# SciML/NeuralPDE.jl

Hardware: AMD Instinct MI355X
Metric: collocation-point residual+grad evals/sec, 2D Poisson 4x64 MLP (higher is better)
Workload: dtype f32, hidden-layer forward / dA / dW GEMMs as 3-piece bf16 split products (6 bf16 MFMAs per product block, fp32 accumulation; 24 mantissa bits rebuilt; the five small piece products on an accumulator of their own: zero-mean, a third of the rms error of an fp32-MFMA fmaf chain per GEMM output, tools/m

## Files before the change

### neuralpde.jl_amd/csrc/pinn_kernels2.hpp

```cpp
#pragma once
#include "pinn_kernels.hpp"

#if defined(PINN_STAMP) && !defined(PINN_EMU)
#define STAMP_MEMBERS unsigned st_acc[24]; unsigned long long st_last;
#define STAMP_INIT(ac) { for (int i_ = 0; i_ < 24; ++i_) (ac).st_acc[i_] = 0; (ac).st_last = __builtin_amdgcn_s_memtime(); }
#define STAMP(i) { const unsigned long long st_now = __builtin_amdgcn_s_memtime(); ac.st_acc[i] += (unsigned)(st_now - ac.st_last); ac.st_last = st_now; }
#define STAMP_EXTRA 128
#else
#define STAMP_MEMBERS
#define STAMP_INIT(ac)
#define STAMP(i)
#define STAMP_EXTRA 0
#endif

#ifndef PINN_F2_REC_LDS
#define PINN_F2_REC_LDS 1
#endif
#ifndef PINN_F2_SWP
#define PINN_F2_SWP 7
#endif
#ifndef PINN_PROBE
#define PINN_PROBE 0
#endif
#ifndef PINN_F2_ADJ_IL
// ... 23 lines not shown

template <class A, class B> struct same_type { static constexpr bool value = false; };
template <class A> struct same_type<A, A> { static constexpr bool value = true; };
template <int HP_, int NHH_, int D_, int NW_, bool WBAR_REG_>
struct Shape2 {
    static constexpr int HP = HP_, MT = HP_ / 16, NHH = NHH_, LH = NHH_ + 1, D = D_, NW = NW_, MTW = MT / NW_;
    static constexpr bool WBAR_REG = WBAR_REG_;
};
template <class SH>
struct Acc2 {
    vfloat4 wbar[(SH::WBAR_REG && SH::NHH > 0) ? SH::NHH : 1][SH::MTW][SH::MT];
    vfloat4 bbar[SH::LH][SH::MTW];
    vfloat4 w1bar[SH::D][SH::MTW];
    vfloat4 wLbar[SH::MTW];
    vfloat bLbar;
    vfloat pbar[MAX_PARAMS];
    vdacc lsum;
    int cur_term;
    STAMP_MEMBERS
};

template <int HP_, int NHH_, int D_, unsigned D1MASK_, unsigned long long PAIRS_, int NPAIR_, int PG_, unsigned HI_ = 0, int GEMM_ = GEMM_SPLIT>
struct Spec2 {
    using J = JetSet<D1MASK_, PAIRS_, NPAIR_, HI_>;
    static constexpr unsigned HI = HI_;
    static constexpr int FAMILY = 2;
    static constexpr int GEMM = GEMM_;
    static constexpr int HP = HP_, MT = HP_ / 16, NHH = NHH_, LH = NHH_ + 1, D = D_, NPAIR = NPAIR_, PG = PG_;
    static constexpr unsigned D1MASK = D1MASK_;
    static constexpr unsigned long long PAIRS = PAIRS_;
    static constexpr int NW = (HP_ >= 128 && J::C * PG_ <= F2_NW8_MAXNG) ? F2_WAVES128 : 4;
// ... 39 lines not shown
    static constexpr int XSZB = BFX ? XSZ_BF : XSZ;
    static constexpr bool BFX_TR = BFX && TR_SHAPE;
    static constexpr bool DW_NATURAL = BFX_TR;
    static constexpr int ZTW = BFX_TR ? 0 : NG * (MT / NW) * 256;
    static constexpr int LDS_UP = (((NW + 1) * NG * 16 + 63) / 64) * 64;
    static_assert(PG_ >= 1 && PG_ <= 4, "one tape wave per point group");
    static constexpr bool CHUNKED = (2 * XSZB + NW * ZTW + LDS_UP) * 4 > 160 * 1024;
    static constexpr int CH_AT = 16 * HP_;
    static constexpr int CH_ZT = MTW * 256;
    static constexpr int CHSZ = CH_AT + NW * CH_ZT;
    static_assert(!CHUNKED || 2 * CHSZ <= XSZ, "chunk double buffer must fit inside X1");
    static constexpr int OFF_X1 = XSZB;
    static constexpr int OFF_ZT = 2 * XSZB;
    static constexpr int OFF_UP = 2 * XSZB + (CHUNKED ? 0 : NW * ZTW);
    static constexpr int LDS_BASE = OFF_UP + LDS_UP;
#ifndef PINN_F2_WG3
#define PINN_F2_WG3 0
#endif
    static constexpr int WG_PER_CU = (NW == 8) ? 1 : ((PINN_F2_WG3 && LDS_BASE * 4 <= 53 * 1024) ? 3 : ((LDS_BASE * 4 <= 80 * 1024) ? 2 : 1));
    static constexpr int RECQ = MT * 256;
    static constexpr int LDS_CAP = (WG_PER_CU == 3 ? 53 : (WG_PER_CU == 2 ? 80 : 160)) * 256 - 64;
    static constexpr int NRQ_ALL = (LH > 2 ? LH - 2 : 0) * NG;
    static constexpr int NRQ_FIT = (LDS_CAP - LDS_BASE) / RECQ;
    static constexpr int NRQ = PINN_F2_REC_LDS ? (NRQ_FIT < NRQ_ALL ? (NRQ_FIT > 0 ? NRQ_FIT : 0) : NRQ_ALL) : 0;
    static constexpr int LDS_WG = LDS_BASE + NRQ * RECQ;
    static constexpr int OCC = WG_PER_CU * NW / 4;
    static constexpr int LDS_FWD = 2 * XSZB + LDS_UP;
    static constexpr int WG_FWD_LDS = (160 * 1024 - 1024) / (LDS_FWD * 4);
    static constexpr int WG_FWD = (WG_FWD_LDS * NW >= 16) ? 16 / NW : (WG_FWD_LDS < 1 ? 1 : WG_FWD_LDS);
    static constexpr int OCC_FWD = WG_FWD * NW / 4;
#ifndef PINN_F2_NO_WBAR_REG
#define PINN_F2_NO_WBAR_REG 0
#endif
    static constexpr bool WBAR_REG = !PINN_F2_NO_WBAR_REG && (NHH_ * MTW * MT * 4 <= 96);
    using Shape = Shape2<HP_, NHH_, D_, NW, WBAR_REG>;
};

template <class S>
DEV void acc2_init(Acc2<typename S::Shape>& ac, const GroupArgs& ga, int blk, int w, bool bwd) {
    constexpr int HP = S::HP, MT = S::MT, MTW = S::MTW, NHH = S::NHH, LH = S::LH, D = S::D;
    const vint lane = lane_id();
    const vint g = lane >> 4;
    const vint c = lane & vint(15);
    float* slab = ga.slabs + (size_t)blk * S::SLAB;
    PINN_UNROLL for (int l = 0; l < ((S::WBAR_REG && NHH > 0) ? NHH : 1); ++l)
        PINN_UNROLL for (int t = 0; t < MTW; ++t)
            PINN_UNROLL for (int ti = 0; ti < MT; ++ti) ac.wbar[l][t][ti] = vzero4();
    if (!S::WBAR_REG && bwd && !ga.chain)
        for (int hl = 0; hl < NHH; ++hl)
            PINN_UNROLL for (int t = 0; t < MTW; ++t)
                PINN_UNROLL for (int ti = 0; ti < MT; ++ti)
                    gstore4(slab + S::O_WBAR, vint((((hl * MT + w * MTW + t) * MT + ti) * 64) * 4) + (lane << 2), vzero4());
    PINN_UNROLL for (int l = 0; l < LH; ++l)
        PINN_UNROLL for (int t = 0; t < MTW; ++t) ac.bbar[l][t] = vzero4();
    PINN_UNROLL for (int i = 0; i < D; ++i)
        PINN_UNROLL for (int t = 0; t < MTW; ++t) ac.w1bar[i][t] = vzero4();
    PINN_UNROLL for (int t = 0; t < MTW; ++t) ac.wLbar[t] = vzero4();
    ac.bLbar = vfloat(0.f);
    PINN_UNROLL for (int i = 0; i < MAX_PARAMS; ++i) ac.pbar[i] = vfloat(0.f);
    ac.lsum = vdacc_zero();
    ac.cur_term = -1;
    STAMP_INIT(ac)
    if (bwd && ga.chain) {
        if (S::WBAR_REG)
            PINN_UNROLL for (int hl = 0; hl < NHH; ++hl)
                PINN_UNROLL for (int t = 0; t < MTW; ++t)
                    PINN_UNROLL for (int ti = 0; ti < MT; ++ti)
                        ac.wbar[hl][t][ti] = gload4(slab + S::O_WBAR, vint((((hl * MT + w * MTW + t) * MT + ti) * 64) * 4) + (lane << 2));
        const vbool c0i = veq(c, 0);
        PINN_UNROLL for (int t = 0; t < MTW; ++t)
            PINN_UNROLL for (int r = 0; r < 4; ++r) {
                const vint n = vint(16 * (w * MTW + t) + r) + (g << 2);
                PINN_UNROLL for (int l = 0; l < LH; ++l) ac.bbar[l][t][r] = gload_masked(slab + S::O_BH + l * HP, n, c0i);
                PINN_UNROLL for (int i = 0; i < D; ++i) ac.w1bar[i][t][r] = gload_masked(slab + S::O_W1 + i * HP, n, c0i);
                ac.wLbar[t][r] = gload_masked(slab + S::O_WL, n, c0i);
            }
        if (w == 0) {
            const vbool l0 = veq(lane, 0);
            ac.bLbar = gload_masked(slab + S::O_BL, lane & vint(0), l0);
            PINN_UNROLL for (int j = 0; j < MAX_PARAMS; ++j) ac.pbar[j] = gload_masked(slab + S::O_P, vint(j) + (lane & vint(0)), l0);
        }
    }
}

template <class S, int MODE, int ACTK>
DEV void wave_tiles2(const GroupArgs& ga, int blk, int nblocks, int w, float* lds, Acc2<typename S::Shape>& ac,
                     int term_lo, int term_hi, int tile_lo, int tile_hi) {
    constexpr int HP = S::HP, MT = S::MT, MTW = S::MTW, NHH = S::NHH, LH = S::LH, D = S::D, C = S::C, PG = S::PG, NG = S::NG;
    constexpr int NFIRST = S::NFIRST;
    using J = typename S::J;
    constexpr bool BWD = (MODE == MODE_FUSED || MODE == MODE_GRADIN || MODE == MODE_GRADREC);
    constexpr bool SUMS = (MODE == MODE_FUSED || MODE == MODE_LOSS);
    constexpr bool TAPE_ONLY = (MODE == MODE_RESID || MODE == MODE_LOSS);
    constexpr bool RECOUT = (MODE == MODE_FWDREC), RECIN = (MODE == MODE_GRADREC);
    constexpr bool IS_FWD = (MODE == MODE_FWD || MODE == MODE_FWDREC), IS_GRADIN = (MODE == MODE_GRADIN || MODE == MODE_GRADREC);
    constexpr bool WPRE = (MT * MTW * 4 <= 16);
    constexpr bool TR_OVL = S::BFX_TR && WPRE && !S::CHUNKED;
    const int wave = blk * S::NW + w;
    const vint lane = lane_id();
    const vint g = lane >> 4;
    const vint c = lane & vint(15);
    const vbool g0 = veq(g, 0);
    const vint sw = S::BFX_TR ? (((g << 4) + (c ^ ((g >> 1) << 2))) << 1) : (lane << 2);
    vint trb[2];
    PINN_UNROLL for (int jh = 0; jh < 2; ++jh) {
        const vint gg = c & vint(3), pc = ((g & vint(1)) << 3) + vint(4 * jh) + (c >> 2);
        trb[jh] = (((gg << 4) + (pc ^ ((gg >> 1) << 2))) << 1);
    }
    vint trbq[2];
    PINN_UNROLL for (int jh = 0; jh < 2; ++jh) trbq[jh] = trb[jh] + (g >> 1) * vint(S::KB * 3 * 256);
    const vbool klo = vlt(g, 2);
    const float* P = ga.packed;
    constexpr int act = ACTK;
    static_assert(ACTK != ACT_MIXED, "per-layer activation kinds are compiled for family 1 (small nets) only");
// ... 3 lines not shown
    const ubuf SB = ub_make(ga.scratch + (size_t)blk * (ga.scr_stride ? ga.scr_stride : S::SCR), S::SCR);
    float* X0 = lds;
    float* X1 = lds + S::OFF_X1;
    float* ZT = lds + S::OFF_ZT + w * S::ZTW;
    float* UP = lds + (BWD ? S::OFF_UP : 2 * S::XSZB);
    float* RL = lds + S::LDS_BASE;
    auto rec_in_lds = [](int layer, int q) { return layer >= 1 && layer <= LH - 2 && (LH - 2 - layer) * NG + q < S::NRQ; };
    auto rl_off = [&](int layer, int q, int t) { return vint((((LH - 2 - layer) * NG + q) * MT + w * MTW + t) * 256) + (lane << 2); };

    float* slab = ga.slabs + (size_t)blk * S::SLAB;
    auto& wbar = ac.wbar;
    auto& bbar = ac.bbar;
    auto& w1bar = ac.w1bar;
    auto& wLbar = ac.wLbar;
    vfloat& bLbar = ac.bLbar;
    auto& pbar = ac.pbar;
    vdacc& lsum = ac.lsum;
    int& cur_term = ac.cur_term;

    auto ld_wf = [&](int hl, int t, int mi) -> vfloat4 {
        return ub_load4(PB, S::OFF_WPK + ((hl * MT + w * MTW + t) * MT + mi) * 256, lane << 2);
    };
    auto ld_wt = [&](int hl, int t, int mo) -> vfloat4 {
        return ub_load4(PB, S::OFF_WTPK + ((hl * MT + w * MTW + t) * MT + mo) * 256, lane << 2);
    };
    auto ld_bias = [&](int layer, int t) -> vfloat4 { return ub_load4(PB, S::off_b(layer) + 16 * (w * MTW + t), g << 2); };

    vfloat4 wL[MTW];
    PINN_UNROLL for (int t = 0; t < MTW; ++t) wL[t] = ub_load4(PB, S::OFF_WL + 16 * (w * MTW + t), g << 2);
    const vbf8 wb_probe = ((PINN_PROBE & 8) && S::BFIMG) ? ub_load_bf8(PB, S::OFF_WB, lane << 2) : vbf8{};
    const float bL = P[S::OFF_BL];

    wave_prio(1);
    const int first = tile_lo + (((blk - tile_lo) % nblocks) + nblocks) % nblocks;
    for (int tix = first; tix < tile_hi; tix += nblocks) {
        STAMP(15)
        int k = term_lo;
        for (int j = term_lo + 1; j < term_hi; ++j)
            if (tix >= ga.terms[j].tile0) k = j;
        if (k != cur_term) {
            if (cur_term >= 0 && SUMS)
                ga.losspart[(size_t)wave * ga.nterms_total + ga.terms[cur_term].term_id] = wave_sum_dd(lsum, g0);
            lsum = vdacc_zero();
            cur_term = k;
        }
        const TermDev& T = ga.terms[k];
        const int pbase = (tix - T.tile0) * S::TP;
        const ubuf RB = ub_make((RECOUT || RECIN) ? ga.rec + (size_t)tix * S::REC : ga.scratch, S::REC);

        vfloat x[PG][D];
        vbool valid[PG];
        PINN_UNROLL for (int pg = 0; pg < PG; ++pg) {
            vint p = vint(pbase + 16 * pg) + c;
            valid[pg] = vlt(p, T.N);
            PINN_UNROLL for (int i = 0; i < D; ++i) x[pg][i] = gload_masked(T.pts, p * T.dt + vint(T.imap[i]), valid[pg]);
        }

// ... 143 lines not shown
                    PINN_UNROLL for (int t = 0; t < MTW; ++t)
                        PINN_UNROLL for (int e = 0; e < 4; ++e) Cc[q][t][e] += Cs[q][t][e];
        };
#ifndef PINN_F2_ACC_2PASS_ALL
#define PINN_F2_ACC_2PASS_ALL 0
#endif
        constexpr bool ACC_2PASS = PINN_F2_ACC_2PASS_ALL || (HP >= 128 && NG >= 5);
        auto acc_mode = [&](int bit) -> int { return (PINN_F2_SPLIT_ACC2 & bit) ? (ACC_2PASS ? 2 : 1) : 0; };

        vfloat4 A[NG][MTW];
        vfloat U[PG][C];
        constexpr int SRC_PRE = 2;
        vfloat srcv[SRC_PRE];
        PINN_UNROLL for (int j = 0; j < SRC_PRE; ++j) srcv[j] = vfloat(0.f);
        vbool valid_w = valid[0];
        PINN_UNROLL for (int pg = 1; pg < PG; ++pg) if (w == pg) valid_w = valid[pg];
        if (!RECIN) {
            PINN_UNROLL for (int t = 0; t < MTW; ++t) {
                const int n0 = 16 * (w * MTW + t);
                vfloat4 b1 = ub_load4(PB, S::off_b(0) + n0, g << 2);
                vfloat4 w1[D];
                PINN_UNROLL for (int i = 0; i < D; ++i) w1[i] = ub_load4(PB, S::OFF_W1 + i * HP + n0, g << 2);
                PINN_UNROLL for (int pg = 0; pg < PG; ++pg) {
                    vfloat4 z = b1;
                    PINN_UNROLL for (int i = 0; i < D; ++i)
                        PINN_UNROLL for (int r = 0; r < 4; ++r) z[r] = vfma(w1[i][r], x[pg][i], z[r]);
                    A[pg * C][t] = z;
                    PINN_UNROLL for (int kf = 0; kf < NFIRST; ++kf) A[pg * C + 1 + kf][t] = w1[S::first_axis(kf)];
                    PINN_UNROLL for (int ch = 1 + NFIRST; ch < C; ++ch) A[pg * C + ch][t] = vzero4();
                }
            }
            act_forward(A, 0);
            STAMP(0)
            PINN_UNROLL for (int hl = 0; hl < NHH; ++hl) {
                float* Xin = (hl & 1) ? X1 : X0;
                vfloat4 wf[WPRE ? MT : 1][MTW], bv[MTW];
                vbf8 wb[S::BFX ? S::KB : 1][S::BFX ? MTW : 1][3];
                if (S::BFX) {
                    PINN_UNROLL for (int t = 0; t < MTW; ++t) bv[t] = ld_bias(hl + 1, t);
                    PINN_UNROLL for (int kb = 0; kb < S::KB; ++kb)
                        PINN_UNROLL for (int t = 0; t < MTW; ++t)
                            PINN_UNROLL for (int sp = 0; sp < 3; ++sp)
                                wb[kb][t][sp] = (PINN_PROBE & 8) ? wb_probe : ub_load_bf8(PB, S::OFF_WB + (((hl * MT + w * MTW + t) * S::KB + kb) * 3 + sp) * 256, lane << 2);
                    sched_fence();
                } else if (WPRE) {
                    PINN_UNROLL for (int mi = 0; mi < MT; ++mi)
                        PINN_UNROLL for (int t = 0; t < MTW; ++t)
                            wf[mi][t] = ld_wf(hl, t, mi);
                    PINN_UNROLL for (int t = 0; t < MTW; ++t) bv[t] = ld_bias(hl + 1, t);
                    sched_fence();
                }
                if (TR_OVL && BWD && hl == 0) wg_barrier();
                publish(Xin, A);
                wg_barrier();
                STAMP(1)
                const bool bias_after = S::BFX && (PINN_F2_SWP & 1) && acc_mode(1) == 2;
                PINN_UNROLL for (int t = 0; t < MTW; ++t) {
                    if (!WPRE && !S::BFX) bv[t] = ld_bias(hl + 1, t);
                    PINN_UNROLL for (int pg = 0; pg < PG; ++pg) {
                        A[pg * C][t] = bias_after ? vzero4() : bv[t];
                        PINN_UNROLL for (int ch = 1; ch < C; ++ch) A[pg * C + ch][t] = vzero4();
                    }
                }
                wave_prio(0);
                if (S::BFX && (PINN_F2_SWP & 1)) {
// ... 45 lines not shown
                        if (j < T.nsrc) srcv[j] = gload_masked(T.src, vint(j * T.N + pbase + 16 * w) + c, valid_w);
            {
                PINN_UNROLL for (int q = 0; q < NG; ++q) {
                    vfloat s = vfloat(0.f);
                    PINN_UNROLL for (int t = 0; t < MTW; ++t)
                        PINN_UNROLL for (int r = 0; r < 4; ++r) s = vfma(wL[t][r], A[q][t][r], s);
                    s = xrow_allsum(s);
                    lds_store(UP, vint((w * NG + q) * 16) + c, s);
                }
                wg_barrier();
            }
            PINN_UNROLL for (int pg = 0; pg < PG; ++pg)
                PINN_UNROLL for (int ch = 0; ch < C; ++ch) {
                    vfloat s = vfloat(0.f);
                    PINN_UNROLL for (int ws = 0; ws < S::NW; ++ws) s = s + lds_load(UP, vint((ws * NG + pg * C + ch) * 16) + c);
                    U[pg][ch] = (ch == 0) ? s + vfloat(bL) : s;
                }
        } else {
            PINN_UNROLL for (int pg = 0; pg < PG; ++pg)
                PINN_UNROLL for (int ch = 0; ch < C; ++ch) U[pg][ch] = vfloat(0.f);
            if (LH == 1) {
                PINN_UNROLL for (int t = 0; t < MTW; ++t) {
                    const int n0 = 16 * (w * MTW + t);
                    vfloat4 b1 = ub_load4(PB, S::off_b(0) + n0, g << 2);
                    vfloat4 w1[D];
                    PINN_UNROLL for (int i = 0; i < D; ++i) w1[i] = ub_load4(PB, S::OFF_W1 + i * HP + n0, g << 2);
                    PINN_UNROLL for (int pg = 0; pg < PG; ++pg) {
                        vfloat4 z = b1;
                        PINN_UNROLL for (int i = 0; i < D; ++i)
                            PINN_UNROLL for (int r = 0; r < 4; ++r) z[r] = vfma(w1[i][r], x[pg][i], z[r]);
                        if (!RECZ) z = act_value4<ACLS>(act, z);
// ... 133 lines not shown
                            const rp::Instr ins = rp::fetch_uniform(prog, q);
                            const vfloat va = tape_get(tv, ins.a), vb = tape_get(tv, ins.b), gq = tape_get(ta, R0 + q);
                            vfloat da, db;
                            if (rp::is_bilinear(ins.code)) rp::adjoint_bilinear<vfloat>(ins, va, vb, gq, da, db);
                            else rp::adjoint<vfloat>(ins.code, va, vb, tape_get(tv, R0 + q), ins.imm, gq, da, db);
                            tape_set(ta, ins.a, tape_get(ta, ins.a) + da);
                            tape_set(ta, ins.b, tape_get(ta, ins.b) + db);
                        }
                        PINN_UNROLL for (int ch = 0; ch < C; ++ch)
                            lds_store(UB, vint((w * C + ch) * 16) + c, vselect(vin, rbar * tape_get(ta, DT + NP + ch), vfloat(0.f)));
                        if (T.src_bar)
                            for (int j = 0; j < T.nsrc; ++j)
                                gstore_masked(T.src_bar, vint(j * T.N + pbase + 16 * w) + c, rbar * tape_get(ta, DT + NP + C + j), vand(vin, g0));
                        for (int j = 0; j < ga.nparams_estim; ++j) {
                            vfloat pj = vselect(vand(g0, vin), rbar * tape_get(ta, DT + j), vfloat(0.f));
                            PINN_UNROLL for (int jj = 0; jj < MAX_PARAMS; ++jj) if (jj == j) pbar[jj] += pj;
                        }
                        }
                    }
                }
                }
            wave_prio(1);
            if (!TAPE_ONLY) {
                if (SPRE && NHH - 1 >= 1) load_record(NHH - 1);
                wg_barrier();
                PINN_UNROLL for (int pg = 0; pg < PG; ++pg)
                    PINN_UNROLL for (int ch = 0; ch < C; ++ch) ubar[pg][ch] = lds_load(UB, vint((pg * C + ch) * 16) + c);
            }
        }
        if (TAPE_ONLY) { wg_barrier(); continue; }
        STAMP(5)
// ... 377 lines not shown
                    const vfloat gz = G[pg * C][t][r];
                    bbar[0][t][r] += gz;
                    PINN_UNROLL for (int i = 0; i < D; ++i) w1bar[i][t][r] = vfma(gz, x[pg][i], w1bar[i][t][r]);
                    PINN_UNROLL for (int kf = 0; kf < NFIRST; ++kf)
                        PINN_UNROLL for (int i = 0; i < D; ++i)
                            if (i == S::first_axis(kf)) w1bar[i][t][r] += G[pg * C + 1 + kf][t][r];
                }
        if (NHH == 0) wg_barrier();
        STAMP(13)
    }
}

template <class S, int PG = S::PG >
DEV void acc2_store(Acc2<typename S::Shape>& ac, const GroupArgs& ga, int blk, int w, float* lds) {
    constexpr int HP = S::HP, MT = S::MT, MTW = S::MTW, NHH = S::NHH, LH = S::LH, D = S::D, NG = S::NG;
    const vint lane = lane_id();
    const vint g = lane >> 4;
    const vint c = lane & vint(15);
    float* slab = ga.slabs + (size_t)blk * S::SLAB;
    float* UP = lds + S::OFF_UP;
    if (S::WBAR_REG)
        PINN_UNROLL for (int hl = 0; hl < NHH; ++hl)
            PINN_UNROLL for (int t = 0; t < MTW; ++t)
                PINN_UNROLL for (int ti = 0; ti < MT; ++ti)
                    gstore4(slab + S::O_WBAR, vint((((hl * MT + w * MTW + t) * MT + ti) * 64) * 4) + (lane << 2), ac.wbar[hl][t][ti]);
    const vbool c0 = veq(c, 0);
    auto reduce_cols = [&](vfloat v) -> vfloat {
        v = row_allsum16(v);
        return v;
    };
    PINN_UNROLL for (int t = 0; t < MTW; ++t)
        PINN_UNROLL for (int r = 0; r < 4; ++r) {
            const vint n = vint(16 * (w * MTW + t) + r) + (g << 2);
            PINN_UNROLL for (int l = 0; l < LH; ++l) gstore_masked(slab + S::O_BH + l * HP, n, reduce_cols(ac.bbar[l][t][r]), c0);
            PINN_UNROLL for (int i = 0; i < D; ++i) gstore_masked(slab + S::O_W1 + i * HP, n, reduce_cols(ac.w1bar[i][t][r]), c0);
            gstore_masked(slab + S::O_WL, n, reduce_cols(ac.wLbar[t][r]), c0);
        }
    static_assert(4 * MAX_PARAMS <= 16, "UB holds the per-wave parameter partials");
    const vbool all = vlt(lane, 64);
    float* UBp = UP + S::NW * NG * 16;
    if (w > 0 && w < PG)
        PINN_UNROLL for (int j = 0; j < MAX_PARAMS; ++j)
            lds_store(UBp, vint(w * MAX_PARAMS + j) + (lane & vint(0)), vfloat((float)wave_sum_d(ac.pbar[j], all)));
    if (PG > 1) wg_barrier();
    if (w == 0) {
        float s = (float)wave_sum_d(ac.bLbar, all);
        gstore_masked(slab + S::O_BL, vint(0), vfloat(s), veq(lane, 0));
        PINN_UNROLL for (int j = 0; j < MAX_PARAMS; ++j) {
            vfloat sp = vfloat((float)wave_sum_d(ac.pbar[j], all));
            PINN_UNROLL for (int ws = 1; ws < PG; ++ws) sp = sp + lds_load(UBp, vint(ws * MAX_PARAMS + j) + (lane & vint(0)));
            gstore_masked(slab + S::O_P, vint(j), sp, veq(lane, 0));
        }
    }
#if defined(PINN_STAMP) && !defined(PINN_EMU)
    STAMP(14)
    if ((threadIdx.x & 63) == 0)
        for (int i = 0; i < 24; ++i) reinterpret_cast<unsigned*>(slab + S::SLAB - 128)[w * 24 + i] = ac.st_acc[i];
#endif
}

template <class S, int MODE, int ACTK>
DEV void wave_main2(const GroupArgs& ga, int blk, int nblocks, int w, float* lds) {
    constexpr bool BWD = (MODE == MODE_FUSED || MODE == MODE_GRADIN || MODE == MODE_GRADREC);
    constexpr bool SUMS = (MODE == MODE_FUSED || MODE == MODE_LOSS);
    const int wave = blk * S::NW + w;
    Acc2<typename S::Shape> ac;
    acc2_init<S>(ac, ga, blk, w, BWD);
    if (SUMS)
        for (int j = 0; j < ga.nterms; ++j) ga.losspart[(size_t)wave * ga.nterms_total + ga.terms[j].term_id] = 0.0;
    wave_tiles2<S, MODE, ACTK>(ga, blk, nblocks, w, lds, ac, 0, ga.nterms, 0, ga.ntiles);
    if (SUMS && ac.cur_term >= 0)
        ga.losspart[(size_t)wave * ga.nterms_total + ga.terms[ac.cur_term].term_id] = wave_sum_dd(ac.lsum, veq(lane_id() >> 4, 0));
    if (!BWD) return;
    acc2_store<S>(ac, ga, blk, w, lds);
}

template <class S0, class S1, int ACTK, int MODE = MODE_FUSED>
DEV void wave_main2m(const GroupArgs& ga, int blk, int nblocks, int w, float* lds) {
    static_assert(same_type<typename S0::Shape, typename S1::Shape>::value, "merged launches need members of one network shape and neuron split");
    static_assert(S0::SLAB == S1::SLAB && S0::PACKED == S1::PACKED, "merged launches share the slab and the packed weight image");
    static_assert(S0::DW_NATURAL == S1::DW_NATURAL && S0::BFX_TR == S1::BFX_TR, "merged launches: one order of the dW tiles in the slab, one exchange-image layout");
    static_assert(MODE == MODE_FUSED || MODE == MODE_LOSS, "merged launches: the fused evaluation and the loss-only evaluation");
    const int wave = blk * S0::NW + w;
    Acc2<typename S0::Shape> ac;
    acc2_init<S0>(ac, ga, blk, w, MODE == MODE_FUSED);
    for (int j = 0; j < ga.nterms; ++j) ga.losspart[(size_t)wave * ga.nterms_total + ga.terms[j].term_id] = 0.0;
    wave_tiles2<S0, MODE, ACTK>(ga, blk, nblocks, w, lds, ac, 0, ga.sub_terms0, 0, ga.sub_tiles0);
    wg_barrier();
    wave_tiles2<S1, MODE, ACTK>(ga, blk, nblocks, w, lds, ac, ga.sub_terms0, ga.nterms, ga.sub_tiles0, ga.ntiles);
    if (ac.cur_term >= 0)
        ga.losspart[(size_t)wave * ga.nterms_total + ga.terms[ac.cur_term].term_id] = wave_sum_dd(ac.lsum, veq(lane_id() >> 4, 0));
    if (MODE != MODE_FUSED) return;
    wg_barrier();
    acc2_store<S0, (S0::PG > S1::PG ? S0::PG : S1::PG)>(ac, ga, blk, w, lds);
}

}
```

### neuralpde.jl_amd/csrc/vec.hpp

```cpp
#pragma once
#ifndef __HIPCC_RTC__
#include <cmath>
#include <cstdint>
#include <cstring>
#include <type_traits>
#endif

#ifdef PINN_EMU
#define DEV inline
#define HD inline
#define PINN_UNROLL
namespace wv {
constexpr int W = 64;
struct vbool { bool v[W]; };
struct vint {
    int v[W];
    vint() {}
    vint(int s) { for (int l = 0; l < W; ++l) v[l] = s; }
};
struct vfloat {
    float v[W];
    vfloat() {}
    vfloat(float s) { for (int l = 0; l < W; ++l) v[l] = s; }
};
// ... 62 lines not shown
inline vfloat vselect(const vbool& m, const vfloat& a, const vfloat& b) { vfloat r; for (int l = 0; l < W; ++l) r.v[l] = m.v[l] ? a.v[l] : b.v[l]; return r; }
inline vint vselect(const vbool& m, const vint& a, const vint& b) { vint r; for (int l = 0; l < W; ++l) r.v[l] = m.v[l] ? a.v[l] : b.v[l]; return r; }
inline vfloat gload(const float* p, const vint& i) { vfloat r; for (int l = 0; l < W; ++l) r.v[l] = p[i.v[l]]; return r; }
inline vfloat gload_masked(const float* p, const vint& i, const vbool& m) { vfloat r; for (int l = 0; l < W; ++l) r.v[l] = m.v[l] ? p[i.v[l]] : 0.f; return r; }
inline void gstore(float* p, const vint& i, const vfloat& x) { for (int l = 0; l < W; ++l) p[i.v[l]] = x.v[l]; }
inline void gstore_masked(float* p, const vint& i, const vfloat& x, const vbool& m) { for (int l = 0; l < W; ++l) if (m.v[l]) p[i.v[l]] = x.v[l]; }
inline vfloat4 gload4(const float* p, const vint& i) { vfloat4 r; for (int k = 0; k < 4; ++k) for (int l = 0; l < W; ++l) r.x[k].v[l] = p[i.v[l] + k]; return r; }
inline void gstore4(float* p, const vint& i, const vfloat4& x) { for (int k = 0; k < 4; ++k) for (int l = 0; l < W; ++l) p[i.v[l] + k] = x.x[k].v[l]; }
struct vtape { vfloat r[32]; };
inline vfloat tape_get(const vtape& t, int i) { return t.r[i]; }
inline void tape_set(vtape& t, int i, const vfloat& x) { t.r[i] = x; }
inline void tape_zero(vtape& t) { for (int i = 0; i < 32; ++i) t.r[i] = vfloat(0.f); }
struct urec16 { int x, y, z, w; };
inline void sched_fence() {}
inline int opaque_lane(int x) { return x; }
template <int N> inline void lds_wait() {}
inline void chain_fence() {}
inline void store_pad() {}
inline void keep_alive(const vfloat4&) {}
inline void wave_prio(int) {}
template <int NGROUPS, int MFMA_PER, int AHEAD, int DS_PER = 1> inline void sched_gemm_prefetch() {}
inline void vsincos(const vfloat& x, vfloat& s, vfloat& c) { for (int l = 0; l < W; ++l) { s.v[l] = std::sin(x.v[l]); c.v[l] = std::cos(x.v[l]); } }
inline urec16 uload16(const void* p) { urec16 r; std::memcpy(&r, p, 16); return r; }
struct urec32 { int v[8]; };
inline urec32 uload32(const void* p) { urec32 r; std::memcpy(&r, p, 32); return r; }
struct ubuf { float* p; };
inline ubuf ub_make(const float* p, size_t) { return ubuf{const_cast<float*>(p)}; }
inline vfloat4 ub_load4(const ubuf& b, int soff, const vint& voff) { vfloat4 r; for (int k = 0; k < 4; ++k) for (int l = 0; l < W; ++l) r.x[k].v[l] = b.p[soff + voff.v[l] + k]; return r; }
inline vfloat4 ub_load4_sc1(const ubuf& b, int soff, const vint& voff) { return ub_load4(b, soff, voff); }
inline void ub_store4(const ubuf& b, int soff, const vint& voff, const vfloat4& x) { for (int k = 0; k < 4; ++k) for (int l = 0; l < W; ++l) b.p[soff + voff.v[l] + k] = x.x[k].v[l]; }
inline vfloat ub_load(const ubuf& b, int soff, const vint& voff) { vfloat r; for (int l = 0; l < W; ++l) r.v[l] = b.p[soff + voff.v[l]]; return r; }
inline vfloat ub_load_sc1(const ubuf& b, int soff, const vint& voff) { return ub_load(b, soff, voff); }
inline void ub_store4_wt(const ubuf& b, const vint& voff, const vfloat4& x) { for (int k = 0; k < 4; ++k) for (int l = 0; l < W; ++l) b.p[voff.v[l] + k] = x.x[k].v[l]; }
inline void gstore_masked_wt(float* p, const vint& i, const vfloat& x, const vbool& m) { for (int l = 0; l < W; ++l) if (m.v[l]) p[i.v[l]] = x.v[l]; }
inline void ustore_wt(double* p, double x) { *p = x; }
inline void ustore_wt(float* p, float x) { *p = x; }
inline float uload_wt(const float* p) { return *p; }
inline double uload_wt(const double* p) { return *p; }
inline vfloat lds_load(const float* p, const vint& i) { return gload(p, i); }
inline void lds_store(float* p, const vint& i, const vfloat& x) { gstore(p, i, x); }
inline vfloat4 lds_load4(const float* p, const vint& i) { return gload4(p, i); }
inline void lds_store4(float* p, const vint& i, const vfloat4& x) { gstore4(p, i, x); }
inline void wave_fence() {}
extern thread_local void (*emu_barrier_hook)(void*);
extern thread_local void* emu_barrier_ctx;
inline void wg_barrier() { if (emu_barrier_hook) emu_barrier_hook(emu_barrier_ctx); }
extern thread_local void (*emu_grid_hook)(void*);
extern thread_local void* emu_grid_ctx;
inline void grid_barrier(unsigned*, unsigned) { if (emu_grid_hook) emu_grid_hook(emu_grid_ctx); }
inline void grid_barrier_wt(unsigned*, unsigned) { if (emu_grid_hook) emu_grid_hook(emu_grid_ctx); }
inline vfloat shfl_xor(const vfloat& a, int m) { vfloat r; for (int l = 0; l < W; ++l) r.v[l] = a.v[l ^ m]; return r; }
inline vfloat row_allsum16(const vfloat& a) {
    vfloat v = a;
    for (int n : {8, 4, 2, 1}) { vfloat r; for (int l = 0; l < W; ++l) r.v[l] = v.v[l] + v.v[(l & ~15) | ((l - n) & 15)]; v = r; }
    return v;
}
inline vfloat xrow_allsum(const vfloat& a) {
    vfloat s, t;
    for (int l = 0; l < W; ++l) s.v[l] = a.v[l & ~16] + a.v[l | 16];
    for (int l = 0; l < W; ++l) t.v[l] = s.v[l & ~32] + s.v[l | 32];
    return t;
}
inline float lane0(const vfloat& a) { return a.v[0]; }
inline double wave_sum_d(const vfloat& a, const vbool& m) { double s = 0; for (int l = 0; l < W; ++l) if (m.v[l]) s += (double)a.v[l]; return s; }
struct vdacc { double v[W]; };
inline vdacc vdacc_zero() { vdacc r; for (int l = 0; l < W; ++l) r.v[l] = 0.0; return r; }
inline vdacc vdacc_fma(const vfloat& a, const vfloat& b, const vdacc& c) { vdacc r; for (int l = 0; l < W; ++l) r.v[l] = std::fma((double)a.v[l], (double)b.v[l], c.v[l]); return r; }
inline double wave_sum_dd(const vdacc& a, const vbool& m) { double s = 0; for (int l = 0; l < W; ++l) if (m.v[l]) s += a.v[l]; return s; }
inline vfloat4 mfma16(const vfloat& a, const vfloat& b, const vfloat4& c) {
    vfloat4 d;
    for (int l = 0; l < W; ++l)
        for (int r = 0; r < 4; ++r) {
            int row = (l >> 4) * 4 + r, col = l & 15;
            float acc = c.x[r].v[l];
            for (int k = 0; k < 4; ++k) acc = std::fmaf(a.v[k * 16 + row], b.v[k * 16 + col], acc);
            d.x[r].v[l] = acc;
        }
    return d;
}
inline vfloat4 vzero4() { vfloat4 z; for (int k = 0; k < 4; ++k) z.x[k] = vfloat(0.f); return z; }
inline uint16_t bf16_bits(float x) {
    uint32_t u;
    std::memcpy(&u, &x, 4);
// ... 175 lines not shown
DEV vfloat gload(const float* p, vint i) { return p[i]; }
DEV vfloat gload_masked(const float* p, vint i, vbool m) { return m ? p[i] : 0.f; }
DEV void gstore(float* p, vint i, vfloat x) { p[i] = x; }
DEV void gstore_masked(float* p, vint i, vfloat x, vbool m) { if (m) p[i] = x; }
DEV vfloat4 gload4(const float* p, vint i) { return *reinterpret_cast<const vfloat4*>(p + i); }
DEV void gstore4(float* p, vint i, vfloat4 x) { *reinterpret_cast<vfloat4*>(p + i) = x; }
#ifndef PINN_TAPE_ROWS
#define PINN_TAPE_ROWS 32
#endif
typedef float vtape __attribute__((ext_vector_type(PINN_TAPE_ROWS)));
DEV vfloat tape_get(const vtape& t, int i) { return t[i]; }
DEV void tape_set(vtape& t, int i, vfloat x) { t[i] = x; }
DEV void tape_zero(vtape& t) { PINN_UNROLL for (int i = 0; i < PINN_TAPE_ROWS; ++i) t[i] = 0.f; }
DEV void sched_fence() { __builtin_amdgcn_sched_barrier(0); }
DEV int opaque_lane(int x) { asm volatile("" : "+v"(x)); return x; }
#ifndef PINN_LDS_WAIT_HOIST
#define PINN_LDS_WAIT_HOIST 1
#endif
#ifndef PINN_CHAIN_FENCE
#define PINN_CHAIN_FENCE 1
#endif
DEV void chain_fence() { if (PINN_CHAIN_FENCE) __builtin_amdgcn_sched_barrier(0); }
template <int N> DEV void lds_wait() {
    static_assert(N >= 0 && N <= 15, "lgkmcnt is a 4-bit counter");
    if (PINN_LDS_WAIT_HOIST) {
        __builtin_amdgcn_s_waitcnt(0xC07F | (N << 8));
        __builtin_amdgcn_sched_barrier(0);
    }
}
#ifndef PINN_STORE_PAD
// ... 65 lines not shown
DEV void opaque_v(int& x) { asm volatile("" : "+v"(x)); }
DEV void opaque_s(int& x) { asm volatile("" : "+s"(x)); }
DEV vfloat ub_load_sc1(ubuf b, int soff, vint voff) {
    return __builtin_bit_cast(float, __builtin_amdgcn_raw_buffer_load_b32(b.r, voff * 4, soff * 4, 16));
}
DEV void ub_store4_wt(ubuf b, vint voff, vfloat4 x) {
    __builtin_amdgcn_raw_buffer_store_b128(__builtin_bit_cast(vuint4, x), b.r, voff * 4, 0, 16);
}
DEV void gstore_masked_wt(float* p, vint i, vfloat x, vbool m) { if (m) __hip_atomic_store(p + i, x, __ATOMIC_RELAXED, __HIP_MEMORY_SCOPE_AGENT); }
DEV void ustore_wt(double* p, double x) { __hip_atomic_store(p, x, __ATOMIC_RELAXED, __HIP_MEMORY_SCOPE_AGENT); }
DEV void ustore_wt(float* p, float x) { __hip_atomic_store(p, x, __ATOMIC_RELAXED, __HIP_MEMORY_SCOPE_AGENT); }
DEV float uload_wt(const float* p) { return __hip_atomic_load(p, __ATOMIC_RELAXED, __HIP_MEMORY_SCOPE_AGENT); }
DEV double uload_wt(const double* p) { return __hip_atomic_load(p, __ATOMIC_RELAXED, __HIP_MEMORY_SCOPE_AGENT); }
DEV vfloat lds_load(const float* p, vint i) { return p[i]; }
DEV void lds_store(float* p, vint i, vfloat x) { p[i] = x; }
DEV vfloat4 lds_load4(const float* p, vint i) { return *reinterpret_cast<const vfloat4*>(p + i); }
DEV void lds_store4(float* p, vint i, vfloat4 x) { *reinterpret_cast<vfloat4*>(p + i) = x; }
DEV void wave_fence() {
    __builtin_amdgcn_fence(__ATOMIC_RELEASE, "wavefront");
    __builtin_amdgcn_wave_barrier();
    __builtin_amdgcn_fence(__ATOMIC_ACQUIRE, "wavefront");
}
#ifndef PINN_PROBE
#define PINN_PROBE 0
#endif
DEV void wg_barrier() { if (!(PINN_PROBE & 4)) __syncthreads(); }
DEV void grid_barrier(unsigned* bar, unsigned target) {
    asm volatile("s_waitcnt vmcnt(0)" ::: "memory");
    __syncthreads();
    if (threadIdx.x == 0) {
// ... 41 lines not shown
    asm volatile("s_nop 1\n\tv_permlane32_swap_b32 %0, %1\n\ts_nop 1" : "+v"(s), "+v"(t));
    return s + t;
}
DEV float lane0(vfloat a) { return __builtin_bit_cast(float, __builtin_amdgcn_readfirstlane(__builtin_bit_cast(int, a))); }
DEV double wave_sum_d(vfloat a, vbool m) {
    double s = m ? (double)a : 0.0;
    PINN_UNROLL for (int o = 32; o >= 1; o >>= 1) s += __shfl_xor(s, o, 64);
    return s;
}
using vdacc = double;
DEV vdacc vdacc_zero() { return 0.0; }
DEV vdacc vdacc_fma(vfloat a, vfloat b, vdacc c) { return __builtin_fma((double)a, (double)b, c); }
DEV double wave_sum_dd(vdacc a, vbool m) {
    double s = m ? a : 0.0;
    PINN_UNROLL for (int o = 32; o >= 1; o >>= 1) s += __shfl_xor(s, o, 64);
    return s;
}
DEV vfloat4 mfma16(vfloat a, vfloat b, vfloat4 c) { return __builtin_amdgcn_mfma_f32_16x16x4f32(a, b, c, 0, 0, 0); }
DEV vfloat4 vzero4() { return vfloat4{0.f, 0.f, 0.f, 0.f}; }
typedef __bf16 vbf4 __attribute__((ext_vector_type(4)));
typedef __bf16 vbf8 __attribute__((ext_vector_type(8)));
#ifndef PINN_SPLIT_PK
#define PINN_SPLIT_PK 1
#endif
typedef __bf16 vbf2_ __attribute__((ext_vector_type(2)));
DEV void split3_bf16(vfloat4 x, vbf4& h, vbf4& m, vbf4& l) {
#if PINN_SPLIT_PK
    PINN_UNROLL for (int q = 0; q < 2; ++q) {
        const vfloat2_ xx = {x[2 * q], x[2 * q + 1]};
        const vbf2_ hb = __builtin_convertvector(xx, vbf2_);
// ... 121 lines not shown
```

Measured before the change: 237.3 million.

## Move parameter-gradient partials to LDS and defer wL loads to cut VGPR pressure

```diff
diff --git a/neuralpde.jl_amd/csrc/pinn_kernels2.hpp b/neuralpde.jl_amd/csrc/pinn_kernels2.hpp
--- a/neuralpde.jl_amd/csrc/pinn_kernels2.hpp
+++ b/neuralpde.jl_amd/csrc/pinn_kernels2.hpp
@@ -61,7 +61,7 @@
     vfloat4 w1bar[SH::D][SH::MTW];
     vfloat4 wLbar[SH::MTW];
     vfloat bLbar;
-    vfloat pbar[MAX_PARAMS];
+    float* pbs;
     vdacc lsum;
     int cur_term;
     STAMP_MEMBERS
@@ -131,16 +131,17 @@
     static constexpr int OFF_ZT = 2 * XSZB;
     static constexpr int OFF_UP = 2 * XSZB + (CHUNKED ? 0 : NW * ZTW);
     static constexpr int LDS_BASE = OFF_UP + LDS_UP;
+    static constexpr int LDS_PB = 4 * MAX_PARAMS * 16;
 #ifndef PINN_F2_WG3
 #define PINN_F2_WG3 0
 #endif
-    static constexpr int WG_PER_CU = (NW == 8) ? 1 : ((PINN_F2_WG3 && LDS_BASE * 4 <= 53 * 1024) ? 3 : ((LDS_BASE * 4 <= 80 * 1024) ? 2 : 1));
+    static constexpr int WG_PER_CU = (NW == 8) ? 1 : ((PINN_F2_WG3 && LDS_BASE * 4 <= 53 * 1024) ? 3 : (((LDS_BASE + LDS_PB) * 4 <= 80 * 1024) ? 2 : 1));
     static constexpr int RECQ = MT * 256;
     static constexpr int LDS_CAP = (WG_PER_CU == 3 ? 53 : (WG_PER_CU == 2 ? 80 : 160)) * 256 - 64;
     static constexpr int NRQ_ALL = (LH > 2 ? LH - 2 : 0) * NG;
-    static constexpr int NRQ_FIT = (LDS_CAP - LDS_BASE) / RECQ;
+    static constexpr int NRQ_FIT = (LDS_CAP - LDS_PB - LDS_BASE) / RECQ;
     static constexpr int NRQ = PINN_F2_REC_LDS ? (NRQ_FIT < NRQ_ALL ? (NRQ_FIT > 0 ? NRQ_FIT : 0) : NRQ_ALL) : 0;
-    static constexpr int LDS_WG = LDS_BASE + NRQ * RECQ;
+    static constexpr int LDS_WG = LDS_BASE + NRQ * RECQ + LDS_PB;
     static constexpr int OCC = WG_PER_CU * NW / 4;
     static constexpr int LDS_FWD = 2 * XSZB + LDS_UP;
     static constexpr int WG_FWD_LDS = (160 * 1024 - 1024) / (LDS_FWD * 4);
@@ -154,7 +155,7 @@
 };
 
 template <class S>
-DEV void acc2_init(Acc2<typename S::Shape>& ac, const GroupArgs& ga, int blk, int w, bool bwd) {
+DEV void acc2_init(Acc2<typename S::Shape>& ac, const GroupArgs& ga, int blk, int w, bool bwd, float* pbs) {
     constexpr int HP = S::HP, MT = S::MT, MTW = S::MTW, NHH = S::NHH, LH = S::LH, D = S::D;
     const vint lane = lane_id();
     const vint g = lane >> 4;
@@ -174,7 +175,9 @@
         PINN_UNROLL for (int t = 0; t < MTW; ++t) ac.w1bar[i][t] = vzero4();
     PINN_UNROLL for (int t = 0; t < MTW; ++t) ac.wLbar[t] = vzero4();
     ac.bLbar = vfloat(0.f);
-    PINN_UNROLL for (int i = 0; i < MAX_PARAMS; ++i) ac.pbar[i] = vfloat(0.f);
+    ac.pbs = pbs;
+    if (bwd && w < 4)
+        PINN_UNROLL for (int i = 0; i < MAX_PARAMS; ++i) lds_store(pbs, vint((w * MAX_PARAMS + i) * 16) + c, vfloat(0.f));
     ac.lsum = vdacc_zero();
     ac.cur_term = -1;
     STAMP_INIT(ac)
@@ -195,7 +198,7 @@
         if (w == 0) {
             const vbool l0 = veq(lane, 0);
             ac.bLbar = gload_masked(slab + S::O_BL, lane & vint(0), l0);
-            PINN_UNROLL for (int j = 0; j < MAX_PARAMS; ++j) ac.pbar[j] = gload_masked(slab + S::O_P, vint(j) + (lane & vint(0)), l0);
+            PINN_UNROLL for (int j = 0; j < MAX_PARAMS; ++j) lds_store_masked(pbs, vint(j * 16) + c, gload_masked(slab + S::O_P, vint(j) + (lane & vint(0)), l0), l0);
         }
     }
 }
@@ -214,7 +217,7 @@
     constexpr bool WPRE = (MT * MTW * 4 <= 16);
     constexpr bool TR_OVL = S::BFX_TR && WPRE && !S::CHUNKED;
     const int wave = blk * S::NW + w;
-    const vint lane = lane_id();
+    const vint lane = lane_id_fresh();
     const vint g = lane >> 4;
     const vint c = lane & vint(15);
     const vbool g0 = veq(g, 0);
@@ -248,7 +251,7 @@
     auto& w1bar = ac.w1bar;
     auto& wLbar = ac.wLbar;
     vfloat& bLbar = ac.bLbar;
-    auto& pbar = ac.pbar;
+    float* pbs = ac.pbs;
     vdacc& lsum = ac.lsum;
     int& cur_term = ac.cur_term;
 
@@ -260,10 +263,11 @@
     };
     auto ld_bias = [&](int layer, int t) -> vfloat4 { return ub_load4(PB, S::off_b(layer) + 16 * (w * MTW + t), g << 2); };
 
-    vfloat4 wL[MTW];
-    PINN_UNROLL for (int t = 0; t < MTW; ++t) wL[t] = ub_load4(PB, S::OFF_WL + 16 * (w * MTW + t), g << 2);
+    auto ld_wL = [&](vfloat4 (&wL)[MTW], vfloat& bL) {
+        PINN_UNROLL for (int t = 0; t < MTW; ++t) wL[t] = ub_load4(PB, S::OFF_WL + 16 * (w * MTW + t), g << 2);
+        bL = ub_load(PB, S::OFF_BL, lane & vint(0));
+    };
     const vbf8 wb_probe = ((PINN_PROBE & 8) && S::BFIMG) ? ub_load_bf8(PB, S::OFF_WB, lane << 2) : vbf8{};
-    const float bL = P[S::OFF_BL];
 
     wave_prio(1);
     const int first = tile_lo + (((blk - tile_lo) % nblocks) + nblocks) % nblocks;
@@ -274,7 +278,7 @@
             if (tix >= ga.terms[j].tile0) k = j;
         if (k != cur_term) {
             if (cur_term >= 0 && SUMS)
-                ga.losspart[(size_t)wave * ga.nterms_total + ga.terms[cur_term].term_id] = wave_sum_dd(lsum, g0);
+                ga.losspart[(size_t)wave * ga.nterms_total + ga.terms[cur_term].term_id] = wave_sum_dd(lsum, g0, lane_id_fresh());
             lsum = vdacc_zero();
             cur_term = k;
         }
@@ -448,6 +452,9 @@
         vfloat srcv[SRC_PRE];
         PINN_UNROLL for (int j = 0; j < SRC_PRE; ++j) srcv[j] = vfloat(0.f);
         vbool valid_w = valid[0];
+        vfloat4 wL[MTW];
+        vfloat bL;
+        if (RECIN || NHH == 0) ld_wL(wL, bL);
         PINN_UNROLL for (int pg = 1; pg < PG; ++pg) if (w == pg) valid_w = valid[pg];
         if (!RECIN) {
             PINN_UNROLL for (int t = 0; t < MTW; ++t) {
@@ -476,13 +483,17 @@
                         PINN_UNROLL for (int t = 0; t < MTW; ++t)
                             PINN_UNROLL for (int sp = 0; sp < 3; ++sp)
                                 wb[kb][t][sp] = (PINN_PROBE & 8) ? wb_probe : ub_load_bf8(PB, S::OFF_WB + (((hl * MT + w * MTW + t) * S::KB + kb) * 3 + sp) * 256, lane << 2);
+                    if (hl == NHH - 1) ld_wL(wL, bL);
                     sched_fence();
                 } else if (WPRE) {
                     PINN_UNROLL for (int mi = 0; mi < MT; ++mi)
                         PINN_UNROLL for (int t = 0; t < MTW; ++t)
                             wf[mi][t] = ld_wf(hl, t, mi);
                     PINN_UNROLL for (int t = 0; t < MTW; ++t) bv[t] = ld_bias(hl + 1, t);
+                    if (hl == NHH - 1) ld_wL(wL, bL);
                     sched_fence();
+                } else if (hl == NHH - 1) {
+                    ld_wL(wL, bL);
                 }
                 if (TR_OVL && BWD && hl == 0) wg_barrier();
                 publish(Xin, A);
@@ -558,7 +569,7 @@
                 PINN_UNROLL for (int ch = 0; ch < C; ++ch) {
                     vfloat s = vfloat(0.f);
                     PINN_UNROLL for (int ws = 0; ws < S::NW; ++ws) s = s + lds_load(UP, vint((ws * NG + pg * C + ch) * 16) + c);
-                    U[pg][ch] = (ch == 0) ? s + vfloat(bL) : s;
+                    U[pg][ch] = (ch == 0) ? s + bL : s;
                 }
         } else {
             PINN_UNROLL for (int pg = 0; pg < PG; ++pg)
@@ -722,7 +733,8 @@
                                 gstore_masked(T.src_bar, vint(j * T.N + pbase + 16 * w) + c, rbar * tape_get(ta, DT + NP + C + j), vand(vin, g0));
                         for (int j = 0; j < ga.nparams_estim; ++j) {
                             vfloat pj = vselect(vand(g0, vin), rbar * tape_get(ta, DT + j), vfloat(0.f));
-                            PINN_UNROLL for (int jj = 0; jj < MAX_PARAMS; ++jj) if (jj == j) pbar[jj] += pj;
+                            const vint at = vint((w * MAX_PARAMS + j) * 16) + (lane_id_fresh() & vint(15));
+                            lds_store_masked(pbs, at, lds_load(pbs, at) + pj, g0);
                         }
                         }
                     }
@@ -1130,7 +1142,7 @@
 template <class S, int PG = S::PG >
 DEV void acc2_store(Acc2<typename S::Shape>& ac, const GroupArgs& ga, int blk, int w, float* lds) {
     constexpr int HP = S::HP, MT = S::MT, MTW = S::MTW, NHH = S::NHH, LH = S::LH, D = S::D, NG = S::NG;
-    const vint lane = lane_id();
+    const vint lane = lane_id_fresh();
     const vint g = lane >> 4;
     const vint c = lane & vint(15);
     float* slab = ga.slabs + (size_t)blk * S::SLAB;
@@ -1155,15 +1167,19 @@
     static_assert(4 * MAX_PARAMS <= 16, "UB holds the per-wave parameter partials");
     const vbool all = vlt(lane, 64);
     float* UBp = UP + S::NW * NG * 16;
+    const vbool g0 = veq(g, 0);
+    auto pbar_of = [&](int j) -> vfloat {
+        return vselect(g0, lds_load(ac.pbs, vint((w * MAX_PARAMS + j) * 16) + c), vfloat(0.f));
+    };
     if (w > 0 && w < PG)
         PINN_UNROLL for (int j = 0; j < MAX_PARAMS; ++j)
-            lds_store(UBp, vint(w * MAX_PARAMS + j) + (lane & vint(0)), vfloat((float)wave_sum_d(ac.pbar[j], all)));
+            lds_store(UBp, vint(w * MAX_PARAMS + j) + (lane & vint(0)), vfloat((float)wave_sum_d(pbar_of(j), all)));
     if (PG > 1) wg_barrier();
     if (w == 0) {
         float s = (float)wave_sum_d(ac.bLbar, all);
         gstore_masked(slab + S::O_BL, vint(0), vfloat(s), veq(lane, 0));
         PINN_UNROLL for (int j = 0; j < MAX_PARAMS; ++j) {
-            vfloat sp = vfloat((float)wave_sum_d(ac.pbar[j], all));
+            vfloat sp = vfloat((float)wave_sum_d(pbar_of(j), all));
             PINN_UNROLL for (int ws = 1; ws < PG; ++ws) sp = sp + lds_load(UBp, vint(ws * MAX_PARAMS + j) + (lane & vint(0)));
             gstore_masked(slab + S::O_P, vint(j), sp, veq(lane, 0));
         }
@@ -1181,12 +1197,12 @@
     constexpr bool SUMS = (MODE == MODE_FUSED || MODE == MODE_LOSS);
     const int wave = blk * S::NW + w;
     Acc2<typename S::Shape> ac;
-    acc2_init<S>(ac, ga, blk, w, BWD);
+    acc2_init<S>(ac, ga, blk, w, BWD, lds + S::LDS_WG - S::LDS_PB);
     if (SUMS)
         for (int j = 0; j < ga.nterms; ++j) ga.losspart[(size_t)wave * ga.nterms_total + ga.terms[j].term_id] = 0.0;
     wave_tiles2<S, MODE, ACTK>(ga, blk, nblocks, w, lds, ac, 0, ga.nterms, 0, ga.ntiles);
     if (SUMS && ac.cur_term >= 0)
-        ga.losspart[(size_t)wave * ga.nterms_total + ga.terms[ac.cur_term].term_id] = wave_sum_dd(ac.lsum, veq(lane_id() >> 4, 0));
+        ga.losspart[(size_t)wave * ga.nterms_total + ga.terms[ac.cur_term].term_id] = wave_sum_dd(ac.lsum, veq(lane_id_fresh() >> 4, 0));
     if (!BWD) return;
     acc2_store<S>(ac, ga, blk, w, lds);
 }
@@ -1199,13 +1215,14 @@
     static_assert(MODE == MODE_FUSED || MODE == MODE_LOSS, "merged launches: the fused evaluation and the loss-only evaluation");
     const int wave = blk * S0::NW + w;
     Acc2<typename S0::Shape> ac;
-    acc2_init<S0>(ac, ga, blk, w, MODE == MODE_FUSED);
+    constexpr int LDS_WG = S0::LDS_WG > S1::LDS_WG ? S0::LDS_WG : S1::LDS_WG;
+    acc2_init<S0>(ac, ga, blk, w, MODE == MODE_FUSED, lds + LDS_WG - S0::LDS_PB);
     for (int j = 0; j < ga.nterms; ++j) ga.losspart[(size_t)wave * ga.nterms_total + ga.terms[j].term_id] = 0.0;
     wave_tiles2<S0, MODE, ACTK>(ga, blk, nblocks, w, lds, ac, 0, ga.sub_terms0, 0, ga.sub_tiles0);
     wg_barrier();
     wave_tiles2<S1, MODE, ACTK>(ga, blk, nblocks, w, lds, ac, ga.sub_terms0, ga.nterms, ga.sub_tiles0, ga.ntiles);
     if (ac.cur_term >= 0)
-        ga.losspart[(size_t)wave * ga.nterms_total + ga.terms[ac.cur_term].term_id] = wave_sum_dd(ac.lsum, veq(lane_id() >> 4, 0));
+        ga.losspart[(size_t)wave * ga.nterms_total + ga.terms[ac.cur_term].term_id] = wave_sum_dd(ac.lsum, veq(lane_id_fresh() >> 4, 0));
     if (MODE != MODE_FUSED) return;
     wg_barrier();
     acc2_store<S0, (S0::PG > S1::PG ? S0::PG : S1::PG)>(ac, ga, blk, w, lds);
diff --git a/neuralpde.jl_amd/csrc/vec.hpp b/neuralpde.jl_amd/csrc/vec.hpp
--- a/neuralpde.jl_amd/csrc/vec.hpp
+++ b/neuralpde.jl_amd/csrc/vec.hpp
@@ -100,6 +100,7 @@
 struct urec16 { int x, y, z, w; };
 inline void sched_fence() {}
 inline int opaque_lane(int x) { return x; }
+inline vint lane_id_fresh() { return lane_id(); }
 template <int N> inline void lds_wait() {}
 inline void chain_fence() {}
 inline void store_pad() {}
@@ -125,6 +126,7 @@
 inline double uload_wt(const double* p) { return *p; }
 inline vfloat lds_load(const float* p, const vint& i) { return gload(p, i); }
 inline void lds_store(float* p, const vint& i, const vfloat& x) { gstore(p, i, x); }
+inline void lds_store_masked(float* p, const vint& i, const vfloat& x, const vbool& m) { gstore_masked(p, i, x, m); }
 inline vfloat4 lds_load4(const float* p, const vint& i) { return gload4(p, i); }
 inline void lds_store4(float* p, const vint& i, const vfloat4& x) { gstore4(p, i, x); }
 inline void wave_fence() {}
@@ -153,6 +155,7 @@
 inline vdacc vdacc_zero() { vdacc r; for (int l = 0; l < W; ++l) r.v[l] = 0.0; return r; }
 inline vdacc vdacc_fma(const vfloat& a, const vfloat& b, const vdacc& c) { vdacc r; for (int l = 0; l < W; ++l) r.v[l] = std::fma((double)a.v[l], (double)b.v[l], c.v[l]); return r; }
 inline double wave_sum_dd(const vdacc& a, const vbool& m) { double s = 0; for (int l = 0; l < W; ++l) if (m.v[l]) s += a.v[l]; return s; }
+inline double wave_sum_dd(const vdacc& a, const vbool& m, const vint&) { return wave_sum_dd(a, m); }
 inline vfloat4 mfma16(const vfloat& a, const vfloat& b, const vfloat4& c) {
     vfloat4 d;
     for (int l = 0; l < W; ++l)
@@ -358,6 +361,11 @@
 DEV void tape_zero(vtape& t) { PINN_UNROLL for (int i = 0; i < PINN_TAPE_ROWS; ++i) t[i] = 0.f; }
 DEV void sched_fence() { __builtin_amdgcn_sched_barrier(0); }
 DEV int opaque_lane(int x) { asm volatile("" : "+v"(x)); return x; }
+DEV vint lane_id_fresh() {
+    int x = (int)__builtin_amdgcn_mbcnt_hi(~0u, __builtin_amdgcn_mbcnt_lo(~0u, 0u));
+    asm volatile("" : "+v"(x));
+    return x & 63;
+}
 #ifndef PINN_LDS_WAIT_HOIST
 #define PINN_LDS_WAIT_HOIST 1
 #endif
@@ -453,6 +461,7 @@
 DEV double uload_wt(const double* p) { return __hip_atomic_load(p, __ATOMIC_RELAXED, __HIP_MEMORY_SCOPE_AGENT); }
 DEV vfloat lds_load(const float* p, vint i) { return p[i]; }
 DEV void lds_store(float* p, vint i, vfloat x) { p[i] = x; }
+DEV void lds_store_masked(float* p, vint i, vfloat x, vbool m) { if (m) p[i] = x; }
 DEV vfloat4 lds_load4(const float* p, vint i) { return *reinterpret_cast<const vfloat4*>(p + i); }
 DEV void lds_store4(float* p, vint i, vfloat4 x) { *reinterpret_cast<vfloat4*>(p + i) = x; }
 DEV void wave_fence() {
@@ -524,6 +533,16 @@
 DEV double wave_sum_dd(vdacc a, vbool m) {
     double s = m ? a : 0.0;
     PINN_UNROLL for (int o = 32; o >= 1; o >>= 1) s += __shfl_xor(s, o, 64);
+    return s;
+}
+DEV double wave_sum_dd(vdacc a, vbool m, vint lane) {
+    double s = m ? a : 0.0;
+    PINN_UNROLL for (int o = 32; o >= 1; o >>= 1) {
+        const unsigned long long u = __builtin_bit_cast(unsigned long long, s);
+        const unsigned lo = (unsigned)__builtin_amdgcn_ds_bpermute((lane ^ o) << 2, (int)(unsigned)u);
+        const unsigned hi = (unsigned)__builtin_amdgcn_ds_bpermute((lane ^ o) << 2, (int)(unsigned)(u >> 32));
+        s += __builtin_bit_cast(double, (unsigned long long)lo | ((unsigned long long)hi << 32));
+    }
     return s;
 }
 DEV vfloat4 mfma16(vfloat a, vfloat b, vfloat4 c) { return __builtin_amdgcn_mfma_f32_16x16x4f32(a, b, c, 0, 0, 0); }
```

Result: slower. 234.7 million (-1.1%).
